# ChainBreak/denoising_diffusion_deep_fake

Hardware: AMD Instinct MI355X
Metric: training images/sec (256x256 U-Net, bs=16/GPU) (higher is better)
Workload: dtype f32; 1 GPU; d3f train_denoiser step: noise blend -> Unet(resnet34) fwd -> (MSE+1-SSIM)/2 -> bwd -> Adam, 256x256 synthetic face crops, bs=16/GPU, random-init weights, train-mode BatchNorm; image_size=256, batch_per_gpu=16, global_batch=16, parallelism=dp1, graph_step=False, adam_overlap_tail=False, adam_overlap_tail_steps=0, ranks_seen=1, csrc_digest=c8a0c545483ee32b

## Files before the change

denoising_diffusion_deep_fake_amd/csrc/c_api.hip:

```cpp
#include "../../include/d3f_hip.h"

#include <cstdarg>
#include <cstdio>
#include <cstring>
#include <new>
#include <vector>

#include "engine.h"
#include "head_act.h"
#include "philox.h"

namespace d3f {
static thread_local char g_err[1024] = "";
int set_error(int code, const char* fmt, ...) {
  va_list ap;
  va_start(ap, fmt);
  vsnprintf(g_err, sizeof(g_err), fmt, ap);
  va_end(ap);
  return code;
}
}

namespace d3f {
struct ProfRec {
// ... 333 lines not shown
  return h->e.export_shape(name, dims);
}

size_t d3f_conv_packed_bytes(int dtype, const d3f_conv_desc* d, int which) {
  ConvLayer L;
  if (plan(L, dtype, d, 0) != 0) return 0;
  if (L.upfold) return which == 0 ? L.wfc : L.wd4 + L.wds;
  return which == 0 ? L.wf : L.wd;
}
int d3f_conv_pack_weights(int dtype, const d3f_conv_desc* d, const float* w, void* w_fwd, void* w_dgrad,
                          void* stream) {
  ConvLayer L;
  if (int rc = plan(L, dtype, d, 0)) return rc;
  if (L.upfold) {
    D3F_CHECK(w_fwd != nullptr && d->CinReal == d->C0 + d->C1, "conv_pack_weights: up-sample folded layer");
    char* wds = w_dgrad && d->C1 > 0 ? reinterpret_cast<char*>(w_dgrad) + L.wd4 : nullptr;
    return pack_up_launch(dtype, w, d->Cout, d->C0, d->C1, w_fwd, L.CoutPad, w_dgrad, L.C0Rows, wds, L.C1Rows,
                          (hipStream_t)stream);
  }
  void* const dst[2] = {w_fwd, w_dgrad};
  PackTable t[2];
  int blocks[2] = {0, 0};
  for (int k = 0; k < 2; ++k) {
    t[k].n = dst[k] != nullptr ? 1 : 0;
    if (t[k].n && (blocks[k] = conv_pack_entry(L, 0, 0, 0, k == 0, k == 1, 0, t[k].e[0])) < 0) return blocks[k];
  }
  for (int k = 0; k < 2; ++k)
    if (int rc = pack_all_launch(dtype, w, dst[k], t[k], blocks[k], (hipStream_t)stream)) return rc;
  return 0;
}
int d3f_conv_upsample_folded(int dtype, const d3f_conv_desc* d) {
  ConvLayer L;
  return (d != nullptr && plan(L, dtype, d, 0) == 0 && L.upfold) ? 1 : 0;
// ... 39 lines not shown
}
size_t d3f_conv_winograd_filter_bytes(const d3f_conv_desc* d) {
  ConvLayer L;
  return (d == nullptr || plan(L, D3F_F32, d, PLAN_FWD) != 0) ? 0 : L.wu;
}
size_t d3f_conv_winograd_stats_floats(const d3f_conv_desc* d, int* tiles) {
  ConvLayer L;
  if (d == nullptr || plan(L, D3F_F32, d, PLAN_FWD) != 0 || L.wu == 0) return 0;
  if (tiles) *tiles = L.wino_rows;
  return (size_t)L.wino_rows * L.CoutPad * 2;
}
int d3f_conv_winograd_pack(const d3f_conv_desc* d, const float* w, void* u, void* stream) {
  ConvLayer L;
  if (int rc = wino_plan(L, d)) return rc;
  D3F_CHECK(w && u && d->CinReal == d->C0, "conv_winograd_pack: null argument or padded input channels");
  return conv_winograd_pack_launch(w, reinterpret_cast<float*>(u), d->Cout, d->C0, (hipStream_t)stream);
}
int d3f_conv_winograd_forward(const d3f_conv_desc* d, const void* src0, const void* u, void* y, float* stats,
                              const float* scale, const float* shift, const void* residual, int relu, void* stream) {
  ConvLayer L;
  if (int rc = wino_plan(L, d)) return rc;
  if (d->B == 0) return 0;
  D3F_CHECK(src0 && u && y && ((scale == nullptr) == (shift == nullptr)), "conv_winograd_forward: null argument");
  D3F_CHECK(scale != nullptr || (residual == nullptr && relu == 0),
            "conv_winograd_forward: residual / ReLU belong to the eval epilogue (scale and shift)");
  ConvFwdBufs b;
  b.src0 = src0; b.w = u; b.out = y;
  if (scale != nullptr) {
    b.scale = scale; b.shift = shift; b.res = residual; b.relu = relu ? 1 : 0;
  } else {
    b.stats = stats;
// ... 501 lines not shown
```

denoising_diffusion_deep_fake_amd/csrc/common.h:

```cpp
#pragma once
#include <hip/hip_runtime.h>
#include <stdint.h>
#include <stddef.h>
#include <stdlib.h>

namespace d3f {

typedef uint16_t bf16_t;

typedef float f32x16 __attribute__((ext_vector_type(16)));
typedef float f32x4 __attribute__((ext_vector_type(4)));
typedef __bf16 bf16x8 __attribute__((ext_vector_type(8)));

}
#ifndef D3F_F32
#define D3F_F32 0
#define D3F_BF16 1
#define D3F_F32X3 2
#endif
namespace d3f {

static inline const char* prof_knob(const char* name) {
#ifdef D3F_PROFILING
  return getenv(name);
// ... 185 lines not shown
  return p;
}

struct ConvTile {
  int BM, BN;
};
int conv_igemm_plan(ConvParams& p, int dtype, bool allow_splitk = false);
size_t conv_splitk_floats(const ConvParams& p);
int conv_igemm_launch(const ConvParams& p, int dtype, hipStream_t stream);
bool conv_igemm_small_c(const ConvParams& p, int dtype);
bool conv_igemm_fast_addr(const ConvParams& p, bool smallc);
bool conv_winograd_fits(const ConvParams& p, int dtype);
bool conv_winograd_applies(const ConvParams& p, int dtype);
int conv_winograd_stat_rows(const ConvParams& p);
size_t conv_winograd_filter_floats(const ConvParams& p);
int conv_winograd_pack_launch(const float* w , float* u, int Cout, int Cin, hipStream_t stream);
int conv_winograd_launch(const ConvParams& p , hipStream_t stream);
bool conv_pres_applies(const ConvParams& p, int dtype);
void conv_pres_plan(ConvParams& p);
int conv_pres_launch(const ConvParams& p, hipStream_t stream);
bool conv_patch_applies(const ConvParams& p, int dtype);
bool conv_stem_applies(const ConvParams& p, int dtype);
bool conv_stem_bf16_applies(const ConvParams& p, int dtype);
void conv_patch_plan(ConvParams& p, int dtype);
int conv_patch_launch(const ConvParams& p, hipStream_t stream);

struct WgradParams {
  const void* dy;
  const void* src0;
  const void* src1;
  float* partial;
// ... 105 lines not shown
  const void* dy = nullptr;
  const void* w = nullptr;
  const void* w_skip = nullptr;
  void* dx0 = nullptr;
  void* dx1 = nullptr;
  int acc0 = 0, acc1 = 0;
  float* slabs = nullptr;
  const void* bn_y = nullptr;
  const float* bn_coef = nullptr;
  float* bn_partial = nullptr;
  const void* bn_a = nullptr;
};
int conv_layer_dgrad(const ConvLayer& L, const ConvDgradBufs& b, hipStream_t s, const NetSplit* ns = nullptr);
struct PackEntry;
int conv_pack_entry(const ConvLayer& L, long w_off, size_t wf_off, size_t wd_off, bool fwd, bool dgrad, uint32_t block0,
                    PackEntry& e);

}
```

denoising_diffusion_deep_fake_amd/csrc/conv_plan.hip:

```cpp
#include "pointwise.h"

#include <algorithm>

namespace d3f {

int conv_layer_plan(ConvLayer& L) {
  D3F_CHECK(L.dtype == D3F_F32 || L.dtype == D3F_BF16 || L.dtype == D3F_F32X3, "conv: dtype %d", L.dtype);
  L.sdtype = L.dtype == D3F_F32X3 ? D3F_F32 : L.dtype;
  const int ve = L.sdtype == D3F_F32 ? 4 : 8, bke = L.sdtype == D3F_F32 ? 32 : 64;
  const size_t wsz = L.dtype == D3F_F32X3 ? 6 : L.sdtype == D3F_F32 ? 4 : 2;
  D3F_CHECK(L.B >= 0 && L.Hv > 0 && L.Wv > 0 && L.C0 > 0 && L.C1 >= 0 && L.Cout > 0, "conv: extent");
  D3F_CHECK(L.C0 % ve == 0 && L.C1 % ve == 0, "conv: channels must be multiples of %d", ve);
  D3F_CHECK(L.KH == L.KW && L.KH >= 1 && L.KH <= 7, "conv: kernel %dx%d", L.KH, L.KW);
  D3F_CHECK(L.stride == 1 || L.stride == 2, "conv: stride %d", L.stride);
  D3F_CHECK(!L.up0 || (L.Hv % 2 == 0 && L.Wv % 2 == 0), "conv: up-sampled extent must be even");
  D3F_CHECK(L.CinReal > 0 && L.CinReal <= L.C0 + L.C1, "conv: CinReal");

  const int B = L.B, K = L.KH;
  L.Cin = L.C0 + L.C1;
  L.Ho = (L.Hv + 2 * L.pad - K) / L.stride + 1;
  L.Wo = (L.Wv + 2 * L.pad - K) / L.stride + 1;
  L.CoutPad = (int)round_up(L.Cout, 16);
  L.Kpad = (int)round_up((long)K * K * L.Cin, bke);
  L.CoutD = (int)round_up(L.Cout, ve);
// ... 145 lines not shown
    const NetSplit nv = net_split_or_single(ns);
    for (int n = 0; n < nv.nets; ++n)
      D3F_HIP(hipMemsetAsync(reinterpret_cast<char*>(b.dx0) + (size_t)n * nv.ws, 0,
                             (size_t)4 * p.M * p.Cout * (L.sdtype == D3F_F32 ? 4 : 2), s));
  }
  if (int rc = conv_igemm_launch(p, L.dtype, s)) return rc;
  if (!L.upfold || L.C1 == 0) return 0;
  ConvParams k = L.dgrad;
  k.src0 = b.dy; k.w = b.w_skip; k.out0 = b.dx1; k.acc0 = b.acc1;
  k.partial = k.splitk > 1 ? b.slabs : nullptr;
  net_conv(k, ns);
  return conv_igemm_launch(k, L.dtype, s);
}

int conv_pack_entry(const ConvLayer& L, long w_off, size_t wf_off, size_t wd_off, bool fwd, bool dgrad, uint32_t block0,
                    PackEntry& e) {
  const int taps = L.KH * L.KW;
  const long nf = fwd ? (long)L.CoutPad * L.Kpad : 0, nd = dgrad ? (long)L.CinRows * L.KpadD : 0;
  D3F_CHECK((!fwd || L.Kpad >= taps * L.Cin) && (!dgrad || L.KpadD >= taps * L.CoutD), "pack_weights: padded K too small");
  const int extent = std::max({L.Cout, L.CinReal, L.Cin, L.CoutPad, L.Kpad, L.CinRows, L.CoutD, L.KpadD});
  D3F_CHECK(extent < 65536 && nf + nd < 0x7fffffffL,
            "pack_weights: the layer exceeds the packing table (extents below 65536, fewer than 2^31 packed elements): "
            "extent %d, %ld elements", extent, nf + nd);
  D3F_CHECK(w_off >= 0 && w_off <= 0xffffffffL && wf_off % 16 == 0 && wd_off % 16 == 0 && (wf_off >> 4) < 0xffffffffull &&
                (wd_off >> 4) < 0xffffffffull,
            "pack_weights: layer out of table range");
  D3F_CHECK(taps <= PACK_LDS_ROW, "pack_weights: %d taps exceed the tile", taps);
  int CT = 32;
  while (CT * taps > PACK_LDS_ROW) CT >>= 1;
  const int crows = std::max(fwd ? L.Cin : 0, dgrad ? L.CinRows : 0);
  const int nrows = std::max(fwd ? L.CoutPad : 0, dgrad ? L.CoutD : 0);
  unsigned mul, shr;
  fast_div_setup((unsigned)taps, &mul, &shr);
  e = PackEntry{};
  e.w_off = (uint32_t)w_off;
  e.wf_off16 = (uint32_t)(wf_off >> 4);
  e.wd_off16 = (uint32_t)(wd_off >> 4);
  e.block0 = block0;
  e.Cout = (uint16_t)L.Cout; e.CinReal = (uint16_t)L.CinReal; e.Cin = (uint16_t)L.Cin;
  e.taps = (uint16_t)taps; e.CoutPad = (uint16_t)L.CoutPad; e.Kpad = (uint16_t)L.Kpad;
  e.CinRows = (uint16_t)L.CinRows; e.CoutD = (uint16_t)L.CoutD; e.KpadD = (uint16_t)L.KpadD;
  e.has_f = fwd ? 1 : 0;
  e.has_d = dgrad ? 1 : 0;
  e.conv_stride = (dgrad && L.parity) ? 2 : 1;
  e.CT = (uint16_t)CT;
  e.ctiles = (uint16_t)((crows + CT - 1) / CT);
  e.taps_mul = mul;
  e.taps_shr = (uint16_t)shr;
  e.ct_log2 = (uint16_t)__builtin_ctz((unsigned)CT);
  return e.ctiles * ((nrows + PACK_NT - 1) / PACK_NT);
}

}
```

denoising_diffusion_deep_fake_amd/csrc/conv_winograd.hip:

```cpp
#include "common.h"

#include <cstdlib>

namespace d3f {

namespace {
constexpr int WCK = 16;
constexpr int WPP = 18;
constexpr int WPB = 4;
typedef float wf32x2 __attribute__((ext_vector_type(2)));

__device__ __forceinline__ int vsw(int row, int ch) { return ch ^ ((row >> 2) & 3); }
}

bool conv_winograd_fits(const ConvParams& p, int dtype) {
  if (dtype != D3F_F32) return false;
  if (p.mode != CONV_RAW_STATS || p.par != 0 || p.KH != 3 || p.KW != 3 || p.stride != 1 || p.pad != 1 || p.C1 != 0 ||
      p.shift0 != 0 || p.zi != 0 || p.Ho != p.Hv || p.Wo != p.Wv || (p.Ho % 16) != 0 || (p.Wo % 16) != 0 ||
      (p.C0 % WCK) != 0 || (p.Cout % 64) != 0 || p.CoutPad < p.Cout)
    return false;
  if ((size_t)p.B * p.Hv * p.Wv * p.C0 * 4 >= (1ull << 31) || (size_t)16 * p.C0 * p.Cout * 4 >= (1ull << 31)) return false;
  return (long)p.B * (p.Ho / 16) * (p.Wo / 16) * (p.Cout / 64) <= 65535L * 4;
}
bool conv_winograd_applies(const ConvParams& p, int dtype) {
  static const bool off = getenv("D3F_NO_WINOGRAD") != nullptr;
  if (off || !conv_winograd_fits(p, dtype)) return false;
  const long wgs = (long)p.B * (p.Ho / 16) * (p.Wo / 16) * (p.Cout / 64) * plan_nets_for(p.plan_nets, 8);
  return wgs >= 256;
}
int conv_winograd_stat_rows(const ConvParams& p) { return p.B * (p.Ho / 16) * (p.Wo / 16); }
size_t conv_winograd_filter_floats(const ConvParams& p) { return (size_t)16 * p.C0 * p.Cout; }

__global__ __launch_bounds__(256) void winograd_pack_kernel(const float* __restrict__ w, float* __restrict__ u, int K, int C) {
  const int id = (int)blockIdx.x * 256 + (int)threadIdx.x;
  if (id >= K * C) return;
  const int k = id / C, c = id - k * C;
  const float* g = w + (long)id * 9;
  float t[4][3];
#pragma unroll
  for (int j = 0; j < 3; ++j) {
    const float g0 = g[j], g1 = g[3 + j], g2 = g[6 + j];
    t[0][j] = g0;
    t[1][j] = 0.5f * (g0 + g1 + g2);
    t[2][j] = 0.5f * (g0 - g1 + g2);
    t[3][j] = g2;
  }
  const long cstride = (long)(C / WCK) * K * WCK;
  float* dst = u + ((long)(c / WCK) * K + k) * WCK + (c % WCK);
#pragma unroll
  for (int i = 0; i < 4; ++i) {
    dst[(4 * i + 0) * cstride] = t[i][0];
    dst[(4 * i + 1) * cstride] = 0.5f * (t[i][0] + t[i][1] + t[i][2]);
    dst[(4 * i + 2) * cstride] = 0.5f * (t[i][0] - t[i][1] + t[i][2]);
    dst[(4 * i + 3) * cstride] = t[i][2];
  }
}

int conv_winograd_pack_launch(const float* w, float* u, int K, int C, hipStream_t stream) {
  D3F_CHECK((C % WCK) == 0 && K > 0 && C > 0, "winograd pack: %d filters x %d channels", K, C);
  hipLaunchKernelGGL(winograd_pack_kernel, dim3((unsigned)cdiv((long)K * C, 256)), dim3(256), 0, stream, w, u, K, C);
  D3F_HIP(hipGetLastError());
  return 0;
}

__global__ __launch_bounds__(256) void conv_winograd_kernel(const ConvParams pin) {
  chain_priority();
  const ConvParams p = conv_params_of_net(pin, (int)blockIdx.z);
  __shared__ __attribute__((aligned(16))) float P[WPP * WPP * WCK];
  __shared__ __attribute__((aligned(16))) float V[2][16 * 64 * WCK];
  const int H = p.Hv, W = p.Wv, C = p.C0, K = p.Cout;
  const int tid = threadIdx.x, lane = tid & 63, wave = tid >> 6;
  const int mt = wave >> 1, nt = wave & 1;
  const int bx = W / 16, by = H / 16;
  const int blk = blockIdx.x;
  const int x0 = (blk % bx) * 16, y0 = ((blk / bx) % by) * 16, b = blk / (bx * by);
  const int n0 = blockIdx.y * 64;
  const __amdgpu_buffer_rsrc_t rx = make_rsrc(p.src0, p.src0_bytes);
  const __amdgpu_buffer_rsrc_t ru = make_rsrc(p.w, p.w_bytes);
// ... 205 lines not shown
```

denoising_diffusion_deep_fake_amd/csrc/engine.hip:

```cpp
#include "engine.h"
#include <vector>

#include "head_act.h"

#include <cstdio>
#include <cstdlib>
#include <cstring>

namespace d3f {

constexpr int CS_PP = 16;
__global__ __launch_bounds__(256) void channel_sum_partial_kernel(const float* __restrict__ x, int C, long HW,
                                                                  float* __restrict__ partial, int nb, long net_in,
                                                                  long net_ws) {
  __shared__ float red[256];
  const int seg = blockIdx.x, c = blockIdx.y, b = (int)blockIdx.z % nb;
  if ((int)blockIdx.z >= nb) {
    net_shift(x, net_in); net_shift(partial, net_ws);
  }
  const float* __restrict__ plane = x + ((long)b * C + c) * HW;
  const long per = (HW + CS_PP - 1) / CS_PP, lo = (long)seg * per, hi = lo + per < HW ? lo + per : HW;
  float s = 0.f;
  if ((HW & 3) == 0 && (per & 3) == 0) {
    for (long i = lo + 4 * threadIdx.x; i < hi; i += 4 * 256) {
// ... 427 lines not shown
  const bool async = !sync_pack && first_late_unit_ > 0;
  const int mid = async ? first_mid_unit_ : -1;
  auto params_of = [&](int n) { return reinterpret_cast<const float*>(reinterpret_cast<const char*>(params0_) + (n ? io->params : 0)); };
  auto ws_of = [&](int n) { return reinterpret_cast<char*>(ws0_) + (size_t)n * net_ws_stride; };
  auto part_of = [&](int ui) { return ui >= first_late_unit_ ? 2 : (mid > 0 && ui >= mid) ? 1 : 0; };
  for (int part = 0; part < 3; ++part) {
    if (part == 1 && mid <= 0) continue;
    PackTable t;
    t.n = 0;
    uint32_t blocks = 0;
    for (int ui = 0; ui < (int)units.size(); ++ui) {
      const Unit& u = units[ui];
      if (first_late_unit_ > 0 && part_of(ui) != part) continue;
      if (first_late_unit_ <= 0 && part != 0) continue;
      if (u.upfold) continue;
      const int nb = conv_pack_entry(u, u.w_off, u.wf_off, u.wd_off, true, u.need_dgrad, blocks, t.e[t.n++]);
      if (nb < 0) return nb;
      blocks += (uint32_t)nb;
    }
    hipStream_t ps = s;
    if (part >= 1 && async) {
      if (int rc = ensure_streams()) return rc;
      if (part == 1 || mid <= 0) {
        D3F_HIP(hipEventRecord(ev_pack_in_, s));
        D3F_HIP(hipStreamWaitEvent(side_, ev_pack_in_, 0));
      }
      ps = side_;
    }
    for (int n = 0; n < nets; ++n) {
      const float* params_ = params_of(n);
      char* ws = ws_of(n);
      if (t.n > 0)
        if (int rc = pack_all_launch(cdtype, params_, ws, t, (int)blocks, ps)) return rc;
      for (int ui = 0; ui < (int)units.size(); ++ui) {
        const Unit& u = units[ui];
        if (!u.wino) continue;
        if (first_late_unit_ > 0 ? part_of(ui) != part : part != 0) continue;
        if (int rc = conv_winograd_pack_launch(params_ + u.w_off, reinterpret_cast<float*>(ws + u.wu_off), u.Cout, u.Cin, ps))
          return rc;
      }
    }
    if (part == 1 && async) {
      D3F_HIP(hipEventRecord(ev_pack_mid_, side_));
      pack_mid_pending_ = true;
    }
    if (part == 2 || (first_late_unit_ <= 0 && part == 0)) {
      for (int n = 0; n < nets; ++n) {
        const float* params_ = params_of(n);
        char* ws = ws_of(n);
        for (const Unit& u : units)
          if (u.upfold)
            if (int rc = pack_up_launch(cdtype, params_ + u.w_off, u.Cout, u.C0, u.C1, ws + u.wfc_off, u.CoutPad,
                                        u.need_dgrad ? ws + u.wd4_off : nullptr, u.C0Rows,
                                        (u.need_dgrad && u.C1 > 0) ? ws + u.wds_off : nullptr, u.C1Rows, ps))
              return rc;
      }
    }
    if (part == 2 && async) {
      D3F_HIP(hipEventRecord(ev_pack_done_, side_));
      pack_pending_ = true;
    }
  }
  return 0;
}

int UnetEngine::forward(const float* params_, float* bnstats, const float* x, float* out, void* ws_,
                        int training, hipStream_t s, const NetIO* io) const {
  char* ws = reinterpret_cast<char*>(ws_);
  D3F_CHECK(nets == 1 || (io != nullptr && training), "unet: the pair engine runs train-mode passes and needs the second "
            "network's offsets");
  NetSplit split{};
// ... 562 lines not shown
```

denoising_diffusion_deep_fake_amd/csrc/pointwise.h:

```cpp
#pragma once
#include <string>

#include "common.h"
#include "philox.h"

namespace d3f {

constexpr int PACK_MAX_LAYERS = 64;

enum BnCoefRow { BN_MEAN, BN_INVSTD, BN_SCALE, BN_SHIFT, BN_K, BN_COEF_ROWS = BN_K + 3 };
inline float* bn_coef(float* block, int C, BnCoefRow row) { return block + (long)row * C; }
inline const float* bn_coef(const float* block, int C, BnCoefRow row) { return block + (long)row * C; }

struct BnEvalEntry {
  uint32_t g_off, b_off, rm_off, rv_off;
  uint32_t coef_off16;
  int32_t C;
};
struct BnEvalTable {
  int n;
  BnEvalEntry e[PACK_MAX_LAYERS];
};
int bn_eval_coeff_all_launch(const float* params, const float* bnstats, void* ws, const BnEvalTable& t,
                             hipStream_t stream);
// ... 178 lines not shown
                               const float stdv[3], uint64_t seed, uint64_t offset, const AffineRngParams* q,
                               hipStream_t stream);
int balanced_index_draw_launch(const int64_t* members, const int64_t* class_start, int Kn, uint64_t seed, uint64_t offset,
                               int64_t* index_out, int B, hipStream_t stream);
__device__ __forceinline__ int64_t balanced_index_rng(uint64_t seed, uint64_t offset, int b,
                                                      const int64_t* __restrict__ members,
                                                      const int64_t* __restrict__ class_start, int Kn) {
  const Philox4 p = rng_block(seed, offset, (uint32_t)b, RNG_G_APPLY);
  const uint32_t j = (uint32_t)(((uint64_t)p.x[1] * (uint32_t)Kn) >> 32);
  const int64_t start = class_start[j], cnt = class_start[j + 1] - start;
  if (cnt <= 0 || cnt >= ((int64_t)1 << 31)) return -1;
  const int64_t m = (int64_t)(((uint64_t)p.x[2] * (uint64_t)cnt) >> 32);
  return members[start + m];
}

int pack_up_launch(int dtype, const float* w, int Cout, int C0, int C1, void* wfc, int CoutPad, void* wd4,
                   int C0Rows, void* wds, int C1Rows, hipStream_t stream);

constexpr int PACK_NT = 32;
constexpr int PACK_LDS_ROW = 288;
struct PackEntry {
  uint32_t w_off;
  uint32_t wf_off16, wd_off16;
  uint32_t block0;
  uint16_t Cout, CinReal, Cin, taps, CoutPad, Kpad, CinRows, CoutD, KpadD, has_d, CT, ctiles;
  uint16_t conv_stride;
  uint16_t has_f;
  uint16_t taps_shr, ct_log2;
  uint32_t taps_mul;
};
struct PackTable {
  int n;
  PackEntry e[PACK_MAX_LAYERS];
};
static_assert(sizeof(PackEntry) == 52, "PackTable travels as a kernel argument: keep its entries small");
int pack_all_launch(int dtype, const float* params, void* ws, const PackTable& t, int blocks,
                    hipStream_t stream);

int noise_blend_launch(const float* x, const float* noise, const float* y_uniform, float lam,
                       float* out, float* r_out, int B, long per_image, hipStream_t stream);
int noise_blend_fixed_launch(const float* x, const float* noise, const float* r, float* out, int B, long per_image,
                             hipStream_t stream);
int noise_blend_rng_launch(const float* x, uint64_t seed, uint64_t offset, float lam, float* out, float* r_out, int B,
                           long per_image, hipStream_t stream);
int noise_blend_fixed_rng_launch(const float* x, uint64_t seed, uint64_t offset, const float* r, float* out, int B,
                                 long per_image, hipStream_t stream);
int noise_blend_fixed_index_rng_launch(const float* x, uint64_t seed, uint64_t offset, const float* r,
                                       const int64_t* index, float* out, int B, long per_image, hipStream_t stream);
int noise_draw_launch(uint64_t seed, uint64_t offset, float* noise, float* y, int B, long per_image,
                      hipStream_t stream);
// ... 36 lines not shown
```

denoising_diffusion_deep_fake_amd/csrc/pointwise.hip:

```cpp
#include "pointwise.h"
#include "philox.h"
#include "vec16.h"

#include <type_traits>

namespace d3f {

template <typename T>
__global__ __launch_bounds__(256) void maxpool_fwd_kernel(const T* __restrict__ in, T* __restrict__ out,
                                                          uint8_t* __restrict__ idx, int B, int H,
                                                          int W, int C, long net_ws) {
  chain_priority();
  if (blockIdx.z != 0) {
    net_shift(in, net_ws); net_shift(out, net_ws); net_shift(idx, net_ws);
  }
  constexpr int N = V16<T>::N;
  const int Ho = H / 2, Wo = W / 2, VC = C / N;
  const long total = (long)B * Ho * Wo * VC;
  for (long i = (long)blockIdx.x * 256 + threadIdx.x; i < total; i += (long)gridDim.x * 256) {
    const int cv = (int)(i % VC);
    long t = i / VC;
    const int ox = (int)(t % Wo);
    t /= Wo;
    const int oy = (int)(t % Ho);
// ... 470 lines not shown
template <typename T, bool X3>
__device__ __forceinline__ void pack_store(T* __restrict__ base, long idx, long plane, float v) {
  if constexpr (X3) {
    const uint32_t xb = __float_as_uint(v), hb = xb & 0xffff0000u;
    const float r1 = v - __uint_as_float(hb);
    const uint32_t mb = __float_as_uint(r1) & 0xffff0000u;
    const float r2 = r1 - __uint_as_float(mb);
    base[idx] = (T)(hb >> 16);
    base[plane + idx] = (T)(mb >> 16);
    base[2 * plane + idx] = (T)(__float_as_uint(r2) >> 16);
  } else {
    base[idx] = from_f32<T>(v);
  }
}

__device__ __forceinline__ unsigned up_fwd_set(int parity, int a) {
  return parity == 0 ? (a == 0 ? 1u : 6u) : (a == 0 ? 3u : 4u);
}
__device__ __forceinline__ unsigned up_bwd_set(int u) { return u == 0 ? 4u : u == 1 ? 6u : u == 2 ? 3u : 1u; }

struct UpDiv {
  unsigned fplane[2], kc[2], c0[2], c1[2], k9[2], cd[2], k4[2];
};
template <typename T, bool X3>
__global__ __launch_bounds__(256) void pack_up_kernel(const float* __restrict__ w, int Cout, int C0, int C1,
                                                      T* __restrict__ wfc, int CoutPad, T* __restrict__ wd4,
                                                      int C0Rows, T* __restrict__ wds, int C1Rows, int CoutD,
                                                      int K9, UpDiv dv) {
  const int Cin = C0 + C1;
  const int Kc = 4 * C0 + 9 * C1, K4 = 16 * CoutD;
  const int nf = 4 * CoutPad * Kc, nd = C0Rows * K4, ns = C1Rows * K9;
  const int fplane = CoutPad * Kc;
  for (int i = (int)blockIdx.x * 256 + (int)threadIdx.x; i < nf + nd + ns; i += (int)gridDim.x * 256) {
    if (i < nf) {
      const int z = fast_div(i, dv.fplane[0], dv.fplane[1]);
      const int r = i - z * fplane;
      const int n = fast_div(r, dv.kc[0], dv.kc[1]), k = r - n * Kc;
      float v = 0.f;
      if (n < Cout) {
        if (k < 4 * C0) {
          const int ab = fast_div(k, dv.c0[0], dv.c0[1]), c = k - ab * C0;
          const unsigned sh = up_fwd_set(z >> 1, ab >> 1), sw = up_fwd_set(z & 1, ab & 1);
          const float* __restrict__ wp = w + ((long)n * Cin + c) * 9;
#pragma unroll
          for (int kh = 0; kh < 3; ++kh)
#pragma unroll
            for (int kw = 0; kw < 3; ++kw)
              if (((sh >> kh) & 1u) && ((sw >> kw) & 1u)) v += wp[kh * 3 + kw];
        } else {
          const int kk = k - 4 * C0, tap = fast_div(kk, dv.c1[0], dv.c1[1]), c1 = kk - tap * C1;
          v = w[((long)n * Cin + C0 + c1) * 9 + tap];
        }
      }
      pack_store<T, X3>(wfc + (X3 ? 3L * z * fplane : (long)z * fplane), r, fplane, v);
    } else if (i >= nf + nd) {
      const int j = i - nf - nd;
      const int c1 = fast_div(j, dv.k9[0], dv.k9[1]), k = j - c1 * K9;
      const int f = fast_div(k, dv.cd[0], dv.cd[1]), n = k - f * CoutD;
      float v = 0.f;
      if (c1 < C1 && n < Cout && f < 9) v = w[((long)n * Cin + C0 + c1) * 9 + (8 - f)];
      pack_store<T, X3>(wds, j, ns, v);
    } else {
      const int j = i - nf;
      const int c = fast_div(j, dv.k4[0], dv.k4[1]), k = j - c * K4;
      const int uv = fast_div(k, dv.cd[0], dv.cd[1]), n = k - uv * CoutD;
      float v = 0.f;
      if (c < C0 && n < Cout) {
        const unsigned sh = up_bwd_set(uv >> 2), sw = up_bwd_set(uv & 3);
        const float* __restrict__ wp = w + ((long)n * Cin + c) * 9;
#pragma unroll
        for (int kh = 0; kh < 3; ++kh)
#pragma unroll
          for (int kw = 0; kw < 3; ++kw)
            if (((sh >> kh) & 1u) && ((sw >> kw) & 1u)) v += wp[kh * 3 + kw];
      }
      pack_store<T, X3>(wd4, j, nd, v);
    }
  }
}

int pack_up_launch(int dtype, const float* w, int Cout, int C0, int C1, void* wfc, int CoutPad, void* wd4,
                   int C0Rows, void* wds, int C1Rows, hipStream_t stream) {
  const int ve = dtype == D3F_BF16 ? 8 : 4;
  const int CoutD = (int)round_up(Cout, ve);
  if (wd4 == nullptr) C0Rows = 0;
  if (wds == nullptr) C1Rows = 0;
  const int K9 = (int)round_up(9L * CoutD, dtype == D3F_BF16 ? 64 : 32);
  const long total = 4L * CoutPad * (4 * C0 + 9 * C1) + (long)C0Rows * 16 * CoutD + (long)C1Rows * K9;
  if (total == 0) return 0;
  D3F_CHECK(total < (1L << 31) - 2048L * 256, "pack_up: %ld elements exceed the 32-bit element index", total);
  UpDiv dv;
  auto setup = [](long d, unsigned (&o)[2]) { fast_div_setup((unsigned)(d > 0 ? d : 1), &o[0], &o[1]); };
  setup((long)CoutPad * (4 * C0 + 9 * C1), dv.fplane);
  setup(4 * C0 + 9 * C1, dv.kc);
  setup(C0, dv.c0);
  setup(C1, dv.c1);
  setup(K9, dv.k9);
  setup(CoutD, dv.cd);
  setup(16 * CoutD, dv.k4);
  if (dtype == D3F_F32)
    hipLaunchKernelGGL((pack_up_kernel<float, false>), dim3(grid_for(total)), dim3(256), 0, stream, w, Cout, C0, C1,
                       (float*)wfc, CoutPad, (float*)wd4, C0Rows, (float*)wds, C1Rows, CoutD, K9, dv);
  else if (dtype == D3F_F32X3)
    hipLaunchKernelGGL((pack_up_kernel<bf16_t, true>), dim3(grid_for(total)), dim3(256), 0, stream, w, Cout, C0, C1,
                       (bf16_t*)wfc, CoutPad, (bf16_t*)wd4, C0Rows, (bf16_t*)wds, C1Rows, CoutD, K9, dv);
  else
    hipLaunchKernelGGL((pack_up_kernel<bf16_t, false>), dim3(grid_for(total)), dim3(256), 0, stream, w, Cout, C0, C1,
                       (bf16_t*)wfc, CoutPad, (bf16_t*)wd4, C0Rows, (bf16_t*)wds, C1Rows, CoutD, K9, dv);
  D3F_HIP(hipGetLastError());
  return 0;
}

template <typename T, bool X3>
__global__ __launch_bounds__(256) void pack_all_kernel(const float* __restrict__ params, char* __restrict__ ws,
                                                       PackTable t) {
  __shared__ float tile[PACK_NT * (PACK_LDS_ROW + 1)];
  int l = 0;
  while (l + 1 < t.n && blockIdx.x >= t.e[l + 1].block0) ++l;
  const PackEntry e = t.e[l];
  const float* __restrict__ w = params + e.w_off;
  T* __restrict__ wf = reinterpret_cast<T*>(ws + (size_t)e.wf_off16 * 16);
  T* __restrict__ wd = reinterpret_cast<T*>(ws + (size_t)e.wd_off16 * 16);
  const int taps = e.taps, Cin = e.Cin, CinReal = e.CinReal, Cout = e.Cout, Kpad = e.Kpad, KpadD = e.KpadD,
// ... 43 lines not shown
      const int nl = i & (PACK_NT - 1), q = i / PACK_NT;
      const int cl = fast_div(q, tmul, tshr), slot = q - cl * taps;
      const int n = n0 + nl, c = c0 + cl;
      if (c < CinRows && n < CoutD)
        pack_store<T, X3>(wd, (long)(unsigned)(c * KpadD + slot * CoutD + n), (long)CinRows * KpadD,
                          tile[nl * stride + cl * taps + (taps - 1 - dgrad_tap_slot_to_flipped(slot, taps, e.conv_stride))]);
    }
    if (nt == 0) {
      const int k0 = taps * CoutD, tail = KpadD - k0;
      for (int i = threadIdx.x; i < CT * tail; i += 256) {
        const int c = c0 + i / tail;
        if (c < CinRows) pack_store<T, X3>(wd, (long)c * KpadD + k0 + i % tail, (long)CinRows * KpadD, 0.f);
      }
    }
  }
}

int pack_all_launch(int dtype, const float* params, void* ws, const PackTable& t, int blocks,
                    hipStream_t stream) {
  if (t.n == 0 || blocks == 0) return 0;
  if (dtype == D3F_F32)
    hipLaunchKernelGGL((pack_all_kernel<float, false>), dim3(blocks), dim3(256), 0, stream, params, (char*)ws, t);
  else if (dtype == D3F_F32X3)
    hipLaunchKernelGGL((pack_all_kernel<bf16_t, true>), dim3(blocks), dim3(256), 0, stream, params, (char*)ws, t);
  else
    hipLaunchKernelGGL((pack_all_kernel<bf16_t, false>), dim3(blocks), dim3(256), 0, stream, params, (char*)ws, t);
  D3F_HIP(hipGetLastError());
  return 0;
}

}
```

Before: 2076 images/sec.

## Fold Winograd and upsample weight packing into batched LDS-tiled pack kernels

```diff
diff --git a/denoising_diffusion_deep_fake_amd/csrc/c_api.hip b/denoising_diffusion_deep_fake_amd/csrc/c_api.hip
--- a/denoising_diffusion_deep_fake_amd/csrc/c_api.hip
+++ b/denoising_diffusion_deep_fake_amd/csrc/c_api.hip
@@ -371,9 +371,12 @@
   if (int rc = plan(L, dtype, d, 0)) return rc;
   if (L.upfold) {
     D3F_CHECK(w_fwd != nullptr && d->CinReal == d->C0 + d->C1, "conv_pack_weights: up-sample folded layer");
-    char* wds = w_dgrad && d->C1 > 0 ? reinterpret_cast<char*>(w_dgrad) + L.wd4 : nullptr;
-    return pack_up_launch(dtype, w, d->Cout, d->C0, d->C1, w_fwd, L.CoutPad, w_dgrad, L.C0Rows, wds, L.C1Rows,
-                          (hipStream_t)stream);
+    UpTable t;
+    t.n = 1;
+    const int blocks = pack_up_entry(dtype, 0, d->Cout, d->C0, d->C1, L.CoutPad, L.C0Rows, L.C1Rows, 0, w_dgrad != nullptr, 0,
+                                     w_dgrad != nullptr && d->C1 > 0, L.wd4, 0, t.e[0]);
+    if (blocks < 0) return blocks;
+    return pack_up_launch(dtype, w, w_fwd, w_dgrad, t, blocks, (hipStream_t)stream);
   }
   void* const dst[2] = {w_fwd, w_dgrad};
   PackTable t[2];
@@ -443,7 +446,12 @@
   ConvLayer L;
   if (int rc = wino_plan(L, d)) return rc;
   D3F_CHECK(w && u && d->CinReal == d->C0, "conv_winograd_pack: null argument or padded input channels");
-  return conv_winograd_pack_launch(w, reinterpret_cast<float*>(u), d->Cout, d->C0, (hipStream_t)stream);
+  D3F_CHECK(reinterpret_cast<uintptr_t>(u) % 16 == 0, "conv_winograd_pack: the filters are stored 16 bytes at a time");
+  PackTable t;
+  t.n = 1;
+  const int blocks = conv_pack_entry(L, 0, 0, 0, false, false, 0, t.e[0], true, 0);
+  if (blocks < 0) return blocks;
+  return pack_all_launch(D3F_F32, w, u, t, blocks, (hipStream_t)stream);
 }
 int d3f_conv_winograd_forward(const d3f_conv_desc* d, const void* src0, const void* u, void* y, float* stats,
                               const float* scale, const float* shift, const void* residual, int relu, void* stream) {
diff --git a/denoising_diffusion_deep_fake_amd/csrc/common.h b/denoising_diffusion_deep_fake_amd/csrc/common.h
--- a/denoising_diffusion_deep_fake_amd/csrc/common.h
+++ b/denoising_diffusion_deep_fake_amd/csrc/common.h
@@ -223,7 +223,6 @@
 bool conv_winograd_applies(const ConvParams& p, int dtype);
 int conv_winograd_stat_rows(const ConvParams& p);
 size_t conv_winograd_filter_floats(const ConvParams& p);
-int conv_winograd_pack_launch(const float* w , float* u, int Cout, int Cin, hipStream_t stream);
 int conv_winograd_launch(const ConvParams& p , hipStream_t stream);
 bool conv_pres_applies(const ConvParams& p, int dtype);
 void conv_pres_plan(ConvParams& p);
@@ -359,6 +358,6 @@
 int conv_layer_dgrad(const ConvLayer& L, const ConvDgradBufs& b, hipStream_t s, const NetSplit* ns = nullptr);
 struct PackEntry;
 int conv_pack_entry(const ConvLayer& L, long w_off, size_t wf_off, size_t wd_off, bool fwd, bool dgrad, uint32_t block0,
-                    PackEntry& e);
-
-}
+                    PackEntry& e, bool wino = false, size_t wu_off = 0);
+
+}
diff --git a/denoising_diffusion_deep_fake_amd/csrc/conv_plan.hip b/denoising_diffusion_deep_fake_amd/csrc/conv_plan.hip
--- a/denoising_diffusion_deep_fake_amd/csrc/conv_plan.hip
+++ b/denoising_diffusion_deep_fake_amd/csrc/conv_plan.hip
@@ -183,7 +183,7 @@
 }
 
 int conv_pack_entry(const ConvLayer& L, long w_off, size_t wf_off, size_t wd_off, bool fwd, bool dgrad, uint32_t block0,
-                    PackEntry& e) {
+                    PackEntry& e, bool wino, size_t wu_off) {
   const int taps = L.KH * L.KW;
   const long nf = fwd ? (long)L.CoutPad * L.Kpad : 0, nd = dgrad ? (long)L.CinRows * L.KpadD : 0;
   D3F_CHECK((!fwd || L.Kpad >= taps * L.Cin) && (!dgrad || L.KpadD >= taps * L.CoutD), "pack_weights: padded K too small");
@@ -195,10 +195,12 @@
                 (wd_off >> 4) < 0xffffffffull,
             "pack_weights: layer out of table range");
   D3F_CHECK(taps <= PACK_LDS_ROW, "pack_weights: %d taps exceed the tile", taps);
+  D3F_CHECK(!wino || (L.wu != 0 && taps == 9 && L.Cin == L.CinReal && wu_off % 16 == 0 && (wu_off >> 4) < 0xffffffffull),
+            "pack_weights: Winograd filters of a layer the kernel does not fit");
   int CT = 32;
   while (CT * taps > PACK_LDS_ROW) CT >>= 1;
-  const int crows = std::max(fwd ? L.Cin : 0, dgrad ? L.CinRows : 0);
-  const int nrows = std::max(fwd ? L.CoutPad : 0, dgrad ? L.CoutD : 0);
+  const int crows = std::max({fwd ? L.Cin : 0, dgrad ? L.CinRows : 0, wino ? L.Cin : 0});
+  const int nrows = std::max({fwd ? L.CoutPad : 0, dgrad ? L.CoutD : 0, wino ? L.Cout : 0});
   unsigned mul, shr;
   fast_div_setup((unsigned)taps, &mul, &shr);
   e = PackEntry{};
@@ -211,6 +213,8 @@
   e.CinRows = (uint16_t)L.CinRows; e.CoutD = (uint16_t)L.CoutD; e.KpadD = (uint16_t)L.KpadD;
   e.has_f = fwd ? 1 : 0;
   e.has_d = dgrad ? 1 : 0;
+  e.has_u = wino ? 1 : 0;
+  e.wu_off16 = wino ? (uint32_t)(wu_off >> 4) : 0;
   e.conv_stride = (dgrad && L.parity) ? 2 : 1;
   e.CT = (uint16_t)CT;
   e.ctiles = (uint16_t)((crows + CT - 1) / CT);
diff --git a/denoising_diffusion_deep_fake_amd/csrc/conv_winograd.hip b/denoising_diffusion_deep_fake_amd/csrc/conv_winograd.hip
--- a/denoising_diffusion_deep_fake_amd/csrc/conv_winograd.hip
+++ b/denoising_diffusion_deep_fake_amd/csrc/conv_winograd.hip
@@ -31,37 +31,6 @@
 int conv_winograd_stat_rows(const ConvParams& p) { return p.B * (p.Ho / 16) * (p.Wo / 16); }
 size_t conv_winograd_filter_floats(const ConvParams& p) { return (size_t)16 * p.C0 * p.Cout; }
 
-__global__ __launch_bounds__(256) void winograd_pack_kernel(const float* __restrict__ w, float* __restrict__ u, int K, int C) {
-  const int id = (int)blockIdx.x * 256 + (int)threadIdx.x;
-  if (id >= K * C) return;
-  const int k = id / C, c = id - k * C;
-  const float* g = w + (long)id * 9;
-  float t[4][3];
-#pragma unroll
-  for (int j = 0; j < 3; ++j) {
-    const float g0 = g[j], g1 = g[3 + j], g2 = g[6 + j];
-    t[0][j] = g0;
-    t[1][j] = 0.5f * (g0 + g1 + g2);
-    t[2][j] = 0.5f * (g0 - g1 + g2);
-    t[3][j] = g2;
-  }
-  const long cstride = (long)(C / WCK) * K * WCK;
-  float* dst = u + ((long)(c / WCK) * K + k) * WCK + (c % WCK);
-#pragma unroll
-  for (int i = 0; i < 4; ++i) {
-    dst[(4 * i + 0) * cstride] = t[i][0];
-    dst[(4 * i + 1) * cstride] = 0.5f * (t[i][0] + t[i][1] + t[i][2]);
-    dst[(4 * i + 2) * cstride] = 0.5f * (t[i][0] - t[i][1] + t[i][2]);
-    dst[(4 * i + 3) * cstride] = t[i][2];
-  }
-}
-
-int conv_winograd_pack_launch(const float* w, float* u, int K, int C, hipStream_t stream) {
-  D3F_CHECK((C % WCK) == 0 && K > 0 && C > 0, "winograd pack: %d filters x %d channels", K, C);
-  hipLaunchKernelGGL(winograd_pack_kernel, dim3((unsigned)cdiv((long)K * C, 256)), dim3(256), 0, stream, w, u, K, C);
-  D3F_HIP(hipGetLastError());
-  return 0;
-}
 
 __global__ __launch_bounds__(256) void conv_winograd_kernel(const ConvParams pin) {
   chain_priority();
diff --git a/denoising_diffusion_deep_fake_amd/csrc/engine.hip b/denoising_diffusion_deep_fake_amd/csrc/engine.hip
--- a/denoising_diffusion_deep_fake_amd/csrc/engine.hip
+++ b/denoising_diffusion_deep_fake_amd/csrc/engine.hip
@@ -465,7 +465,7 @@
       if (first_late_unit_ > 0 && part_of(ui) != part) continue;
       if (first_late_unit_ <= 0 && part != 0) continue;
       if (u.upfold) continue;
-      const int nb = conv_pack_entry(u, u.w_off, u.wf_off, u.wd_off, true, u.need_dgrad, blocks, t.e[t.n++]);
+      const int nb = conv_pack_entry(u, u.w_off, u.wf_off, u.wd_off, true, u.need_dgrad, blocks, t.e[t.n++], u.wino, u.wu_off);
       if (nb < 0) return nb;
       blocks += (uint32_t)nb;
     }
@@ -483,29 +483,25 @@
       char* ws = ws_of(n);
       if (t.n > 0)
         if (int rc = pack_all_launch(cdtype, params_, ws, t, (int)blocks, ps)) return rc;
-      for (int ui = 0; ui < (int)units.size(); ++ui) {
-        const Unit& u = units[ui];
-        if (!u.wino) continue;
-        if (first_late_unit_ > 0 ? part_of(ui) != part : part != 0) continue;
-        if (int rc = conv_winograd_pack_launch(params_ + u.w_off, reinterpret_cast<float*>(ws + u.wu_off), u.Cout, u.Cin, ps))
-          return rc;
-      }
     }
     if (part == 1 && async) {
       D3F_HIP(hipEventRecord(ev_pack_mid_, side_));
       pack_mid_pending_ = true;
     }
     if (part == 2 || (first_late_unit_ <= 0 && part == 0)) {
-      for (int n = 0; n < nets; ++n) {
-        const float* params_ = params_of(n);
-        char* ws = ws_of(n);
-        for (const Unit& u : units)
-          if (u.upfold)
-            if (int rc = pack_up_launch(cdtype, params_ + u.w_off, u.Cout, u.C0, u.C1, ws + u.wfc_off, u.CoutPad,
-                                        u.need_dgrad ? ws + u.wd4_off : nullptr, u.C0Rows,
-                                        (u.need_dgrad && u.C1 > 0) ? ws + u.wds_off : nullptr, u.C1Rows, ps))
-              return rc;
-      }
+      UpTable ut;
+      ut.n = 0;
+      uint32_t ublocks = 0;
+      for (const Unit& u : units) {
+        if (!u.upfold) continue;
+        D3F_CHECK(ut.n < PACK_UP_MAX, "pack_weights: more than %d folded layers", PACK_UP_MAX);
+        const int nb = pack_up_entry(cdtype, u.w_off, u.Cout, u.C0, u.C1, u.CoutPad, u.C0Rows, u.C1Rows, u.wfc_off,
+                                     u.need_dgrad, u.wd4_off, u.need_dgrad && u.C1 > 0, u.wds_off, ublocks, ut.e[ut.n++]);
+        if (nb < 0) return nb;
+        ublocks += (uint32_t)nb;
+      }
+      for (int n = 0; n < nets; ++n)
+        if (int rc = pack_up_launch(cdtype, params_of(n), ws_of(n), ws_of(n), ut, (int)ublocks, ps)) return rc;
     }
     if (part == 2 && async) {
       D3F_HIP(hipEventRecord(ev_pack_done_, side_));
diff --git a/denoising_diffusion_deep_fake_amd/csrc/pointwise.h b/denoising_diffusion_deep_fake_amd/csrc/pointwise.h
--- a/denoising_diffusion_deep_fake_amd/csrc/pointwise.h
+++ b/denoising_diffusion_deep_fake_amd/csrc/pointwise.h
@@ -216,8 +216,23 @@
   return members[start + m];
 }
 
-int pack_up_launch(int dtype, const float* w, int Cout, int C0, int C1, void* wfc, int CoutPad, void* wd4,
-                   int C0Rows, void* wds, int C1Rows, hipStream_t stream);
+constexpr int PACK_UP_MAX = 16;
+struct UpEntry {
+  uint32_t w_off;
+  uint32_t wfc_off16, wd4_off16, wds_off16;
+  uint32_t block0;
+  uint16_t Cout, C0, C1, CoutPad, CoutD, K9;
+  uint16_t C0Rows, C1Rows;
+  uint16_t ct0, ctiles;
+};
+struct UpTable {
+  int n;
+  UpEntry e[PACK_UP_MAX];
+};
+static_assert(sizeof(UpTable) + 3 * sizeof(void*) <= 4096, "UpTable travels as a kernel argument");
+int pack_up_entry(int dtype, long w_off, int Cout, int C0, int C1, int CoutPad, int C0Rows, int C1Rows, size_t wfc_off,
+                  bool wd4, size_t wd4_off, bool wds, size_t wds_off, uint32_t block0, UpEntry& e);
+int pack_up_launch(int dtype, const float* params, void* ws_f, void* ws_d, const UpTable& t, int blocks, hipStream_t stream);
 
 constexpr int PACK_NT = 32;
 constexpr int PACK_LDS_ROW = 288;
@@ -230,12 +245,15 @@
   uint16_t has_f;
   uint16_t taps_shr, ct_log2;
   uint32_t taps_mul;
+  uint32_t wu_off16;
+  uint32_t has_u;
 };
 struct PackTable {
   int n;
   PackEntry e[PACK_MAX_LAYERS];
 };
-static_assert(sizeof(PackEntry) == 52, "PackTable travels as a kernel argument: keep its entries small");
+static_assert(sizeof(PackEntry) == 60, "PackTable travels as a kernel argument: keep its entries small");
+static_assert(sizeof(PackTable) + 2 * sizeof(void*) <= 4096, "PackTable travels as a kernel argument");
 int pack_all_launch(int dtype, const float* params, void* ws, const PackTable& t, int blocks,
                     hipStream_t stream);
 
diff --git a/denoising_diffusion_deep_fake_amd/csrc/pointwise.hip b/denoising_diffusion_deep_fake_amd/csrc/pointwise.hip
--- a/denoising_diffusion_deep_fake_amd/csrc/pointwise.hip
+++ b/denoising_diffusion_deep_fake_amd/csrc/pointwise.hip
@@ -508,99 +508,149 @@
   }
 }
 
-__device__ __forceinline__ unsigned up_fwd_set(int parity, int a) {
+__host__ __device__ constexpr unsigned up_fwd_set(int parity, int a) {
   return parity == 0 ? (a == 0 ? 1u : 6u) : (a == 0 ? 3u : 4u);
 }
-__device__ __forceinline__ unsigned up_bwd_set(int u) { return u == 0 ? 4u : u == 1 ? 6u : u == 2 ? 3u : 1u; }
-
-struct UpDiv {
-  unsigned fplane[2], kc[2], c0[2], c1[2], k9[2], cd[2], k4[2];
-};
+__host__ __device__ constexpr unsigned up_bwd_set(int u) { return u == 0 ? 4u : u == 1 ? 6u : u == 2 ? 3u : 1u; }
+__device__ __forceinline__ float up_sum(const float (&g)[9], unsigned sh, unsigned sw) {
+  float v = 0.f;
+#pragma unroll
+  for (int kh = 0; kh < 3; ++kh)
+#pragma unroll
+    for (int kw = 0; kw < 3; ++kw)
+      if (((sh >> kh) & 1u) && ((sw >> kw) & 1u)) v += g[kh * 3 + kw];
+  return v;
+}
+
+constexpr int PACK_UP_NT = 16;
+constexpr int PACK_UP_CT = 32;
 template <typename T, bool X3>
-__global__ __launch_bounds__(256) void pack_up_kernel(const float* __restrict__ w, int Cout, int C0, int C1,
-                                                      T* __restrict__ wfc, int CoutPad, T* __restrict__ wd4,
-                                                      int C0Rows, T* __restrict__ wds, int C1Rows, int CoutD,
-                                                      int K9, UpDiv dv) {
-  const int Cin = C0 + C1;
-  const int Kc = 4 * C0 + 9 * C1, K4 = 16 * CoutD;
-  const int nf = 4 * CoutPad * Kc, nd = C0Rows * K4, ns = C1Rows * K9;
-  const int fplane = CoutPad * Kc;
-  for (int i = (int)blockIdx.x * 256 + (int)threadIdx.x; i < nf + nd + ns; i += (int)gridDim.x * 256) {
-    if (i < nf) {
-      const int z = fast_div(i, dv.fplane[0], dv.fplane[1]);
-      const int r = i - z * fplane;
-      const int n = fast_div(r, dv.kc[0], dv.kc[1]), k = r - n * Kc;
-      float v = 0.f;
-      if (n < Cout) {
-        if (k < 4 * C0) {
-          const int ab = fast_div(k, dv.c0[0], dv.c0[1]), c = k - ab * C0;
-          const unsigned sh = up_fwd_set(z >> 1, ab >> 1), sw = up_fwd_set(z & 1, ab & 1);
-          const float* __restrict__ wp = w + ((long)n * Cin + c) * 9;
-#pragma unroll
-          for (int kh = 0; kh < 3; ++kh)
-#pragma unroll
-            for (int kw = 0; kw < 3; ++kw)
-              if (((sh >> kh) & 1u) && ((sw >> kw) & 1u)) v += wp[kh * 3 + kw];
-        } else {
-          const int kk = k - 4 * C0, tap = fast_div(kk, dv.c1[0], dv.c1[1]), c1 = kk - tap * C1;
-          v = w[((long)n * Cin + C0 + c1) * 9 + tap];
-        }
+__global__ __launch_bounds__(256) void pack_up_kernel(const float* __restrict__ params, char* __restrict__ ws_f,
+                                                      char* __restrict__ ws_d, UpTable t) {
+  constexpr int NT = PACK_UP_NT, CT = PACK_UP_CT, run = CT * 9, stride = run + 1;
+  __shared__ float tile[NT * stride];
+  int l = 0;
+  while (l + 1 < t.n && blockIdx.x >= t.e[l + 1].block0) ++l;
+  const UpEntry e = t.e[l];
+  const float* __restrict__ w = params + e.w_off;
+  const int Cout = e.Cout, C0 = e.C0, C1 = e.C1, CoutPad = e.CoutPad, CoutD = e.CoutD, Cin = C0 + C1;
+  const int rel = (int)(blockIdx.x - e.block0);
+  const int nt = rel / e.ctiles, ct = rel % e.ctiles;
+  const bool skip = ct >= e.ct0;
+  const int n0 = nt * NT, c0 = (skip ? ct - e.ct0 : ct) * CT, Csrc = skip ? C1 : C0;
+  constexpr int LU = 9;
+  const unsigned cbase = (unsigned)((skip ? C0 : 0) + c0);
+  for (int i0 = threadIdx.x; i0 < NT * run; i0 += 256 * LU) {
+    float v[LU];
+    int dst[LU];
+#pragma unroll
+    for (int u = 0; u < LU; ++u) {
+      const int i = i0 + u * 256;
+      const int nl = i / run, r = i - nl * run;
+      const int n = n0 + nl, c = c0 + r / 9;
+      dst[u] = i < NT * run ? nl * stride + r : -1;
+      const bool real = dst[u] >= 0 && n < Cout && c < Csrc;
+      const float x = w[real ? ((unsigned)n * (unsigned)Cin + cbase) * 9u + (unsigned)r : 0u];
+      v[u] = real ? x : 0.f;
+    }
+#pragma unroll
+    for (int u = 0; u < LU; ++u)
+      if (dst[u] >= 0) tile[dst[u]] = v[u];
+  }
+  __syncthreads();
+  T* __restrict__ wfc = reinterpret_cast<T*>(ws_f + (size_t)e.wfc_off16 * 16);
+  const int Kc = 4 * C0 + 9 * C1;
+  const long fplane = (long)CoutPad * Kc;
+  for (int i = threadIdx.x; i < NT * CT; i += 256) {
+    const int cl = i & (CT - 1), nl = i / CT;
+    const int n = n0 + nl, c = c0 + cl;
+    if (n >= CoutPad || c >= Csrc) continue;
+    float g[9];
+#pragma unroll
+    for (int k = 0; k < 9; ++k) g[k] = tile[nl * stride + cl * 9 + k];
+    const long row = (long)n * Kc;
+#pragma unroll
+    for (int z = 0; z < 4; ++z) {
+      T* __restrict__ base = wfc + (X3 ? 3L * z * fplane : (long)z * fplane);
+      if (!skip) {
+#pragma unroll
+        for (int ab = 0; ab < 4; ++ab)
+          pack_store<T, X3>(base, row + ab * C0 + c, fplane,
+                            up_sum(g, up_fwd_set(z >> 1, ab >> 1), up_fwd_set(z & 1, ab & 1)));
+      } else {
+#pragma unroll
+        for (int tap = 0; tap < 9; ++tap) pack_store<T, X3>(base, row + 4 * C0 + tap * C1 + c, fplane, g[tap]);
       }
-      pack_store<T, X3>(wfc + (X3 ? 3L * z * fplane : (long)z * fplane), r, fplane, v);
-    } else if (i >= nf + nd) {
-      const int j = i - nf - nd;
-      const int c1 = fast_div(j, dv.k9[0], dv.k9[1]), k = j - c1 * K9;
-      const int f = fast_div(k, dv.cd[0], dv.cd[1]), n = k - f * CoutD;
-      float v = 0.f;
-      if (c1 < C1 && n < Cout && f < 9) v = w[((long)n * Cin + C0 + c1) * 9 + (8 - f)];
-      pack_store<T, X3>(wds, j, ns, v);
+    }
+  }
+  const int Rows = skip ? e.C1Rows : e.C0Rows;
+  const int Kd = skip ? e.K9 : 16 * CoutD;
+  T* __restrict__ wd = reinterpret_cast<T*>(ws_d + (size_t)(skip ? e.wds_off16 : e.wd4_off16) * 16);
+  const long dplane = (long)Rows * Kd;
+  for (int i = threadIdx.x; i < NT * CT; i += 256) {
+    const int nl = i & (NT - 1), cl = i / NT;
+    const int n = n0 + nl, c = c0 + cl;
+    if (c >= Rows || n >= CoutD) continue;
+    float g[9];
+#pragma unroll
+    for (int k = 0; k < 9; ++k) g[k] = tile[nl * stride + cl * 9 + k];
+    const long at = (long)c * Kd + n;
+    if (!skip) {
+#pragma unroll
+      for (int uv = 0; uv < 16; ++uv)
+        pack_store<T, X3>(wd, at + uv * CoutD, dplane, up_sum(g, up_bwd_set(uv >> 2), up_bwd_set(uv & 3)));
     } else {
-      const int j = i - nf;
-      const int c = fast_div(j, dv.k4[0], dv.k4[1]), k = j - c * K4;
-      const int uv = fast_div(k, dv.cd[0], dv.cd[1]), n = k - uv * CoutD;
-      float v = 0.f;
-      if (c < C0 && n < Cout) {
-        const unsigned sh = up_bwd_set(uv >> 2), sw = up_bwd_set(uv & 3);
-        const float* __restrict__ wp = w + ((long)n * Cin + c) * 9;
-#pragma unroll
-        for (int kh = 0; kh < 3; ++kh)
-#pragma unroll
-          for (int kw = 0; kw < 3; ++kw)
-            if (((sh >> kh) & 1u) && ((sw >> kw) & 1u)) v += wp[kh * 3 + kw];
-      }
-      pack_store<T, X3>(wd4, j, nd, v);
-    }
-  }
-}
-
-int pack_up_launch(int dtype, const float* w, int Cout, int C0, int C1, void* wfc, int CoutPad, void* wd4,
-                   int C0Rows, void* wds, int C1Rows, hipStream_t stream) {
+#pragma unroll
+      for (int f = 0; f < 9; ++f) pack_store<T, X3>(wd, at + f * CoutD, dplane, g[8 - f]);
+    }
+  }
+  if (skip && nt == 0) {
+    const int k0 = 9 * CoutD, tail = Kd - k0;
+    for (int i = threadIdx.x; i < CT * tail; i += 256) {
+      const int c = c0 + i / tail;
+      if (c < Rows) pack_store<T, X3>(wd, (long)c * Kd + k0 + i % tail, dplane, 0.f);
+    }
+  }
+}
+
+int pack_up_entry(int dtype, long w_off, int Cout, int C0, int C1, int CoutPad, int C0Rows, int C1Rows, size_t wfc_off,
+                  bool wd4, size_t wd4_off, bool wds, size_t wds_off, uint32_t block0, UpEntry& e) {
   const int ve = dtype == D3F_BF16 ? 8 : 4;
   const int CoutD = (int)round_up(Cout, ve);
-  if (wd4 == nullptr) C0Rows = 0;
-  if (wds == nullptr) C1Rows = 0;
+  if (!wd4) C0Rows = 0;
+  if (!wds || C1 == 0) C1Rows = 0;
   const int K9 = (int)round_up(9L * CoutD, dtype == D3F_BF16 ? 64 : 32);
   const long total = 4L * CoutPad * (4 * C0 + 9 * C1) + (long)C0Rows * 16 * CoutD + (long)C1Rows * K9;
-  if (total == 0) return 0;
-  D3F_CHECK(total < (1L << 31) - 2048L * 256, "pack_up: %ld elements exceed the 32-bit element index", total);
-  UpDiv dv;
-  auto setup = [](long d, unsigned (&o)[2]) { fast_div_setup((unsigned)(d > 0 ? d : 1), &o[0], &o[1]); };
-  setup((long)CoutPad * (4 * C0 + 9 * C1), dv.fplane);
-  setup(4 * C0 + 9 * C1, dv.kc);
-  setup(C0, dv.c0);
-  setup(C1, dv.c1);
-  setup(K9, dv.k9);
-  setup(CoutD, dv.cd);
-  setup(16 * CoutD, dv.k4);
+  D3F_CHECK(Cout > 0 && C0 > 0 && C1 >= 0 && CoutPad >= Cout, "pack_up: %d filters (%d rows) x %d + %d channels", Cout,
+            CoutPad, C0, C1);
+  D3F_CHECK(std::max({CoutPad, CoutD, C0 + C1, C0Rows, C1Rows, K9}) < 65536 && total < 0x7fffffffL,
+            "pack_up: the layer exceeds the packing table (extents below 65536, fewer than 2^31 packed elements): %ld elements",
+            total);
+  D3F_CHECK(w_off >= 0 && w_off <= 0xffffffffL && wfc_off % 16 == 0 && (wfc_off >> 4) < 0xffffffffull &&
+                (!C0Rows || (wd4_off % 16 == 0 && (wd4_off >> 4) < 0xffffffffull)) &&
+                (!C1Rows || (wds_off % 16 == 0 && (wds_off >> 4) < 0xffffffffull)),
+            "pack_up: layer out of table range");
+  e = UpEntry{};
+  e.w_off = (uint32_t)w_off;
+  e.wfc_off16 = (uint32_t)(wfc_off >> 4);
+  e.wd4_off16 = C0Rows ? (uint32_t)(wd4_off >> 4) : 0;
+  e.wds_off16 = C1Rows ? (uint32_t)(wds_off >> 4) : 0;
+  e.block0 = block0;
+  e.Cout = (uint16_t)Cout; e.C0 = (uint16_t)C0; e.C1 = (uint16_t)C1; e.CoutPad = (uint16_t)CoutPad;
+  e.CoutD = (uint16_t)CoutD; e.K9 = (uint16_t)K9; e.C0Rows = (uint16_t)C0Rows; e.C1Rows = (uint16_t)C1Rows;
+  e.ct0 = (uint16_t)cdiv(std::max(C0, C0Rows), PACK_UP_CT);
+  e.ctiles = (uint16_t)(e.ct0 + cdiv(std::max(C1, C1Rows), PACK_UP_CT));
+  return e.ctiles * (int)cdiv(std::max(CoutPad, C0Rows || C1Rows ? CoutD : 0), PACK_UP_NT);
+}
+
+int pack_up_launch(int dtype, const float* params, void* ws_f, void* ws_d, const UpTable& t, int blocks, hipStream_t stream) {
+  if (t.n == 0 || blocks == 0) return 0;
   if (dtype == D3F_F32)
-    hipLaunchKernelGGL((pack_up_kernel<float, false>), dim3(grid_for(total)), dim3(256), 0, stream, w, Cout, C0, C1,
-                       (float*)wfc, CoutPad, (float*)wd4, C0Rows, (float*)wds, C1Rows, CoutD, K9, dv);
+    hipLaunchKernelGGL((pack_up_kernel<float, false>), dim3(blocks), dim3(256), 0, stream, params, (char*)ws_f, (char*)ws_d, t);
   else if (dtype == D3F_F32X3)
-    hipLaunchKernelGGL((pack_up_kernel<bf16_t, true>), dim3(grid_for(total)), dim3(256), 0, stream, w, Cout, C0, C1,
-                       (bf16_t*)wfc, CoutPad, (bf16_t*)wd4, C0Rows, (bf16_t*)wds, C1Rows, CoutD, K9, dv);
+    hipLaunchKernelGGL((pack_up_kernel<bf16_t, true>), dim3(blocks), dim3(256), 0, stream, params, (char*)ws_f, (char*)ws_d, t);
   else
-    hipLaunchKernelGGL((pack_up_kernel<bf16_t, false>), dim3(grid_for(total)), dim3(256), 0, stream, w, Cout, C0, C1,
-                       (bf16_t*)wfc, CoutPad, (bf16_t*)wd4, C0Rows, (bf16_t*)wds, C1Rows, CoutD, K9, dv);
+    hipLaunchKernelGGL((pack_up_kernel<bf16_t, false>), dim3(blocks), dim3(256), 0, stream, params, (char*)ws_f, (char*)ws_d, t);
   D3F_HIP(hipGetLastError());
   return 0;
 }
@@ -674,11 +724,51 @@
       }
     }
   }
+  if constexpr (std::is_same_v<T, float> && !X3) {
+    if (e.has_u) {
+      float* __restrict__ wu = reinterpret_cast<float*>(ws + (size_t)e.wu_off16 * 16);
+      const long cstride = (long)Cin * Cout;
+      for (int i = threadIdx.x; i < PACK_NT * 8; i += 256) {
+        const int cl = 4 * (i & 7), nl = i >> 3;
+        const int k = n0 + nl, c = c0 + cl;
+        if (k >= Cout || c >= Cin) continue;
+        float o[16][4];
+#pragma unroll
+        for (int m = 0; m < 4; ++m) {
+          const float* g = tile + nl * stride + (cl + m) * 9;
+          float tm[4][3];
+#pragma unroll
+          for (int j = 0; j < 3; ++j) {
+            const float g0 = g[j], g1 = g[3 + j], g2 = g[6 + j];
+            tm[0][j] = g0;
+            tm[1][j] = 0.5f * (g0 + g1 + g2);
+            tm[2][j] = 0.5f * (g0 - g1 + g2);
+            tm[3][j] = g2;
+          }
+#pragma unroll
+          for (int r = 0; r < 4; ++r) {
+            o[4 * r + 0][m] = tm[r][0];
+            o[4 * r + 1][m] = 0.5f * (tm[r][0] + tm[r][1] + tm[r][2]);
+            o[4 * r + 2][m] = 0.5f * (tm[r][0] - tm[r][1] + tm[r][2]);
+            o[4 * r + 3][m] = tm[r][2];
+          }
+        }
+        float* dst = wu + ((long)(c / 16) * Cout + k) * 16 + (c % 16);
+#pragma unroll
+        for (int pos = 0; pos < 16; ++pos)
+          *reinterpret_cast<float4*>(dst + pos * cstride) = make_float4(o[pos][0], o[pos][1], o[pos][2], o[pos][3]);
+      }
+    }
+  }
 }
 
 int pack_all_launch(int dtype, const float* params, void* ws, const PackTable& t, int blocks,
                     hipStream_t stream) {
   if (t.n == 0 || blocks == 0) return 0;
+  for (int l = 0; l < t.n; ++l)
+    D3F_CHECK(!t.e[l].has_u || (dtype == D3F_F32 && t.e[l].taps == 9 && t.e[l].CT == 32 && t.e[l].Cin == t.e[l].CinReal &&
+                                t.e[l].Cin % 16 == 0),
+              "pack_weights: Winograd filters are made of fp32 3x3 layers with whole 16-channel chunks");
   if (dtype == D3F_F32)
     hipLaunchKernelGGL((pack_all_kernel<float, false>), dim3(blocks), dim3(256), 0, stream, params, (char*)ws, t);
   else if (dtype == D3F_F32X3)
```

Result: no change. 2083 images/sec (median of 6 runs) (+0.4%).
